# JialeTao/MRFA

Measured on AMD Instinct MI355X. Metric: frames/sec (256x256 source+driving pair) fwd+bwd, higher is better.
Workload: dtype f32; 1 GPU; vox1.yaml MTIA (TokenPose_B) prior + DenseMotion + RaftFlow refinement, 256x256, bs=8/GPU, fwd+bwd+clip+Adam, train-mode BN, surrogate L1 loss; global_batch=8, parallelism=dp1, prior=mtia, background_predictor=False, sync_bn=False, launch=hipGraph, optimizer=FlatAdam (K20), mfma=bf16x6

## Files before the change

### mrfa_amd/build.py

```python
import glob
import os
import subprocess
import sys

HERE = os.path.dirname(os.path.abspath(__file__))
ROOT = os.path.dirname(HERE)
CSRC = os.path.join(HERE, "csrc")
LIBDIR = os.path.join(HERE, "_lib")
LIB = os.path.join(LIBDIR, "libmrfa_hip.so")
SOURCES = ["error.cpp", "conv_plan.hip", "conv_mfma.hip", "conv_split.hip", "conv_halo.hip", "conv_small.hip", "conv_lean.hip", "wgrad_mfma.hip", "wgrad_split.hip", "wgrad_halo.hip", "wgrad_small.hip", "wgrad_lean.hip", "conv_fewout.hip", "conv_fewout3.hip", "layout.hip", "pack_multi.hip", "norm.hip", "sample.hip", "elementwise.hip", "optim.hip", "tokenpose.hip", "attention_mfma.hip", "losses.hip", "prior.hip", "pose.hip", "metrics.hip", "frames.hip"]
FLAGS = ["--offload-arch=gfx950", "-O3", "-std=c++17", "-fPIC", "-I" + os.path.join(ROOT, "include"), "-I" + CSRC,
         "-Wno-unused-result"]


def _stale(out, deps):
    if not os.path.exists(out):
        return True
    t = os.path.getmtime(out)
    return any(os.path.getmtime(d) > t for d in deps)


def build(force: bool = False, verbose: bool = True) -> str:
    os.makedirs(LIBDIR, exist_ok=True)
    hipcc = os.environ.get("HIPCC", "/opt/rocm/bin/hipcc")
    headers = [os.path.join(ROOT, "include", "mrfa_hip.h")] + sorted(glob.glob(os.path.join(CSRC, "*.h")))
    objs = []
    procs = []
    for src in SOURCES:
        sp = os.path.join(CSRC, src)
        if not os.path.exists(sp):
            raise FileNotFoundError(sp)
        obj = os.path.join(LIBDIR, os.path.splitext(src)[0] + ".o")
        objs.append(obj)
        if force or _stale(obj, [sp] + headers):
            cmd = [hipcc] + FLAGS + (["-x", "hip"] if src.endswith(".cpp") else []) + ["-c", sp, "-o", obj]
            if verbose:
                print("[mrfa_amd.build]", " ".join(cmd), flush=True)
            procs.append((src, subprocess.Popen(cmd)))
    for src, pr in procs:
        if pr.wait() != 0:
            raise RuntimeError(f"hipcc failed on {src}")
    if force or _stale(LIB, objs):
        cmd = [hipcc, "--offload-arch=gfx950", "-shared", "-fPIC", "-o", LIB] + objs
        if verbose:
            print("[mrfa_amd.build]", " ".join(cmd), flush=True)
        subprocess.check_call(cmd)
    return LIB


if __name__ == "__main__":
    build(force="--force" in sys.argv)
    print(LIB)
```

### mrfa_amd/csrc/common.h

```cpp
#pragma once
#include <hip/hip_runtime.h>
#include <stdio.h>
#include <string.h>
#include "mrfa_hip.h"

typedef float f32x16 __attribute__((ext_vector_type(16)));
typedef float f32x4 __attribute__((ext_vector_type(4)));

void mrfa_set_error(const char* fmt, ...);

struct MrfaTuning {
    int conv_small_env;
    int conv_small;
    int conv_halo, conv_halo_min_tiles, conv_halo_pr, conv_halo_phase, conv_halo_bn256, conv_halo_bn192, conv_halo_bn64_fill;
    int conv_lean, conv_lean_min_wgs, conv_lean_geo, gemm_lean;
    int wgrad_halo, wgrad_halo_min_wgs, wgrad_halo_target_wgs, wgrad_halo_phase, wgrad_lean;
    int conv_fewout3, attention_mfma, split_target_256;
};
extern MrfaTuning g_tune;

struct HaloGeo { int PR, BN; bool phase; };

enum class ConvFamily { lean, gemm_lean, small, halo, halo_dgrad, rows_split, rows_f32, refused };
struct ConvPlan {
    ConvFamily family;
    char error[256];
    long long M;
    int KT;
    int lean_geo, gemm_cfg, small_tm, small_tn;
    HaloGeo halo;
    int BM, BN, splitk;
    bool w8;
    bool fused;
    bool fin_in_launch;
    bool reads_w;
    int last_config;
    bool groups_ok, bst_ok, stride2_ok, mask_ok, phase_dgrad_ok;
};
ConvPlan plan_conv(const mrfa_conv_params& p);

enum class WgradFamily { lean, small, halo, tiled, refused };
struct WgradPlan {
    WgradFamily family;
    char error[192];
    long long M;
    bool lean, small;
    bool groups_ok, stride2_ok;
};
WgradPlan plan_wgrad(const mrfa_wgrad_params& p);

int mrfa_conv_split_launch(hipStream_t st, const mrfa_conv_params& p, int KT, long long M, int splitk, int BN);
bool mrfa_conv_halo_eligible(const mrfa_conv_params& p, HaloGeo* geo);
int mrfa_conv_halo_launch(hipStream_t st, const mrfa_conv_params& p, const HaloGeo& geo);
int mrfa_wgrad_split_launch(hipStream_t st, const mrfa_wgrad_params& p, dim3 grid, long long M, long long kps, int tiles_n, int nsplit, int inner,
                            int total_splits, int taps, long long partial_stride, int BM, int BN);

bool mrfa_wgrad_halo_eligible(const mrfa_wgrad_params& p);
int mrfa_wgrad_halo_launch(hipStream_t st, const mrfa_wgrad_params& p);

bool mrfa_fewout3_wgrad(hipStream_t st, const float* x, int ldx, int N, int H, int W, int Cin, const float* dy, int lddy, int Cout, int R, int pad,
                        float* dw, float* dbias, int* rc);

int mrfa_conv_lean_pick(const mrfa_conv_params& p);
int mrfa_conv_lean_launch(hipStream_t st, const mrfa_conv_params& p, int geo);
int mrfa_gemm_lean_pick(const mrfa_conv_params& p, long long M);
int mrfa_gemm_lean_launch(hipStream_t st, const mrfa_conv_params& p, long long M, int cfg);

bool mrfa_conv_small_eligible(const mrfa_conv_params& p, long long M);
int mrfa_conv_small_launch(hipStream_t st, const mrfa_conv_params& p, long long M, int tm, int tn);

bool mrfa_attention_mfma_ok(int d, int n, const void* qkv, int ld, const void* out, int ldo, const void* dout, int lddo, const void* dqkv, int lddq);
int mrfa_attention_fwd_mfma(hipStream_t st, const float* qkv, int ld, int B, int n, int heads, int d, float scale, float* out, int ldo, float* lse);
int mrfa_attention_bwd_mfma(hipStream_t st, const float* qkv, int ld, const float* out, int ldo, const float* dout, int lddo, const float* lse,
                            float* delta, int B, int n, int heads, int d, float scale, float* dqkv, int lddq);

bool mrfa_wgrad_lean_eligible(const mrfa_wgrad_params& p);
int mrfa_wgrad_lean_multi(hipStream_t st, const mrfa_wgrad_params* ps, int n, unsigned char* taken);

bool mrfa_wgrad_small_eligible(const mrfa_wgrad_params& p, long long M);
int mrfa_wgrad_small_launch(hipStream_t st, const mrfa_wgrad_params& p, long long M);

#define MRFA_CHECK_ARG(cond, ...)                      \
    do {                                               \
        if (!(cond)) {                                 \
            mrfa_set_error(__VA_ARGS__);               \
            return 1;                                  \
        }                                              \
    } while (0)

#define MRFA_CHECK_LAUNCH(name)                                                   \
    do {                                                                          \
        hipError_t e_ = hipGetLastError();                                        \
        if (e_ != hipSuccess) {                                                   \
            mrfa_set_error("%s: launch failed: %s", name, hipGetErrorString(e_)); \
            return 2;                                                             \
        }                                                                         \
    } while (0)

static inline bool aligned16(const void* p) { return (reinterpret_cast<uintptr_t>(p) & 15u) == 0; }
static inline int cdiv(long long a, long long b) { return (int)((a + b - 1) / b); }

static inline int stream_grid(long long work_items, int block) {
    long long g = (work_items + block - 1) / block;
    if (g < 1) g = 1;
    if (g > 256 * 16) g = 256 * 16;
    return (int)g;
}

__device__ __forceinline__ int xcd_tile_index() {
    const int per_xcd = (int)gridDim.x >> 3;
    return (int)(blockIdx.x & 7) * per_xcd + (int)(blockIdx.x >> 3);
}

__device__ __forceinline__ void chain_prio() {
    __builtin_amdgcn_s_setprio(3);
}

__device__ __forceinline__ int stat_group(const mrfa_conv_params& p, long long row, long long M) {
    return p.groups > 1 ? (int)(row / (M / p.groups)) : 0;
}
__device__ __forceinline__ double* stat_slot(const mrfa_conv_params& p, int group, unsigned slot) {
    return p.stats + ((size_t)group * MRFA_STATS_SLOTS + slot % MRFA_STATS_SLOTS) * 2 * p.Cout;
}
static inline long long group_rows(const mrfa_conv_params& p, long long M) {
    if (p.groups <= 1) return M;
    return (p.N % p.groups) == 0 ? M / p.groups : 0;
}

__device__ __forceinline__ bool splitk_last_arriver(unsigned* ticket, unsigned nsplit) {
    __shared__ unsigned s_sk_ticket;
    asm volatile("s_waitcnt vmcnt(0)" ::: "memory");
    __syncthreads();
    if (threadIdx.x == 0) s_sk_ticket = __hip_atomic_fetch_add(ticket, 1u, __ATOMIC_RELAXED, __HIP_MEMORY_SCOPE_AGENT);
    __syncthreads();
    return s_sk_ticket == nsplit - 1;
}

__device__ __forceinline__ bool fin_last_arriver(unsigned* counter, unsigned participants, int idx) {
    __shared__ unsigned s_fin_ticket;
    asm volatile("s_waitcnt vmcnt(0)" ::: "memory");
    __syncthreads();
    if (threadIdx.x == 0) {
        if (idx < 0) {
            s_fin_ticket = __hip_atomic_fetch_add(counter, 1u, __ATOMIC_RELAXED, __HIP_MEMORY_SCOPE_AGENT) == participants - 1;
        } else {
            const unsigned nsh = participants < 8u ? participants : 8u, sh = (unsigned)idx % nsh;
            const unsigned mine = participants / nsh + (sh < participants % nsh ? 1u : 0u);
            unsigned last = 0;
            if (__hip_atomic_fetch_add(counter + 1 + sh, 1u, __ATOMIC_RELAXED, __HIP_MEMORY_SCOPE_AGENT) == mine - 1)
                last = __hip_atomic_fetch_add(counter, 1u, __ATOMIC_RELAXED, __HIP_MEMORY_SCOPE_AGENT) == nsh - 1;
            s_fin_ticket = last;
        }
    }
    __syncthreads();
    return s_fin_ticket != 0;
}

__device__ __forceinline__ double fin_slot_sum(const double* first, size_t stride) {
    double v[MRFA_STATS_SLOTS];
#pragma unroll
    for (int s = 0; s < MRFA_STATS_SLOTS; ++s) v[s] = __hip_atomic_load(first + (size_t)s * stride, __ATOMIC_RELAXED, __HIP_MEMORY_SCOPE_AGENT);
    double t = 0.0;
#pragma unroll
    for (int s = 0; s < MRFA_STATS_SLOTS; ++s) t += v[s];
    return t;
}

__device__ __forceinline__ void fused_bn_finalize(const mrfa_conv_params& p, unsigned participants, int idx = -1, double* scratch = nullptr, int scratch_n = 0) {
    if (!fin_last_arriver(p.fin_counter, participants, idx)) return;
    const double cnt = (double)p.fin_count;
    const int G = p.groups > 1 ? p.groups : 1;
    const int C2 = 2 * p.Cout;
    const bool par = scratch != nullptr && scratch_n >= G * C2;
    if (par) {
        for (int o = threadIdx.x; o < G * C2; o += blockDim.x) scratch[o] = fin_slot_sum(p.stats + (size_t)(o / C2) * MRFA_STATS_SLOTS * C2 + o % C2, (size_t)C2);
        __syncthreads();
    }
    for (int c = threadIdx.x; c < p.Cout; c += blockDim.x) {
        float rm = p.fin_rmean ? p.fin_rmean[c] : 0.f, rv = p.fin_rmean ? p.fin_rvar[c] : 0.f;
        for (int g = 0; g < G; ++g) {
            const double* sg = p.stats + (size_t)g * MRFA_STATS_SLOTS * C2;
            const double t1 = par ? scratch[g * C2 + c] : fin_slot_sum(sg + c, (size_t)C2);
            const double t2 = par ? scratch[g * C2 + p.Cout + c] : fin_slot_sum(sg + p.Cout + c, (size_t)C2);
            const double m = t1 / cnt;
            double var = t2 / cnt - m * m;
            if (var < 0.0) var = 0.0;
            const float mean = (float)m, invstd = (float)(1.0 / sqrt(var + (double)p.fin_eps));
            const double unb = p.fin_count > 1 ? var * cnt / (cnt - 1.0) : var;
            rm = (1.f - p.fin_momentum) * rm + p.fin_momentum * mean;
            rv = (1.f - p.fin_momentum) * rv + p.fin_momentum * (float)unb;
            const float sc = p.fin_gamma[c] * invstd;
            const int gc = g * p.Cout + c;
            p.fin_scale[gc] = sc;
            p.fin_shift[gc] = p.fin_beta[c] - mean * sc;
            if (p.fin_mean) p.fin_mean[gc] = mean;
            if (p.fin_invstd) p.fin_invstd[gc] = invstd;
        }
        if (p.fin_rmean) { p.fin_rmean[c] = rm; p.fin_rvar[c] = rv; }
    }
}

__device__ __forceinline__ float wave_sum(float v) {
#pragma unroll
    for (int o = 32; o > 0; o >>= 1) v += __shfl_xor(v, o, 64);
    return v;
}
```

### mrfa_amd/csrc/conv_mfma.hip

```cpp
#include "common.h"
#include <stdlib.h>

namespace {

constexpr int BK = 32;
constexpr int LDK = BK + 4;

template <int BM, int BN, int WAVES_M, int WAVES_N, bool FLAT>
__global__ __launch_bounds__(WAVES_M * WAVES_N * 64) void conv_mfma_kernel(const mrfa_conv_params p, const int KT, const int kt_per_split,
                                                       const long long M, const int tiles_n, const int total_tiles) {
    constexpr int TM = BM / WAVES_M / 32;
    constexpr int TN = BN / WAVES_N / 32;
    constexpr int NT = WAVES_M * WAVES_N * 64;
    constexpr int RSTEP = NT / 8;
    constexpr int RA = BM / RSTEP;
    constexpr int RB = BN / RSTEP;
    static_assert(WAVES_M * WAVES_N == 4 || WAVES_M * WAVES_N == 8, "4 or 8 waves");
    static_assert(RA >= 1 && RB >= 1, "tile too small for the workgroup");
    static_assert(TM >= 1 && TN >= 1, "tile");

    __shared__ __attribute__((aligned(16))) float smem[2 * (BM + BN) * LDK];

    const int tid = threadIdx.x;
    const int lane = tid & 63;
// ... 35 lines not shown
    bool b_ok[RB];
#pragma unroll
    for (int j = 0; j < RB; ++j) b_ok[j] = (n0 + lrow + RSTEP * j) < p.w_rows;

    f32x4 ra[RA], rb[RB];

    int l_r = 0, l_s = 0, l_c = 0;
    const float* l_w = w;
    const int a_koff = kq * 4;

    auto load_tiles = [&](int kt) {
        if constexpr (!FLAT) {
            const int c0 = l_c * 32 + a_koff;
            f32x4 sc = {1.f, 1.f, 1.f, 1.f}, sh = {0.f, 0.f, 0.f, 0.f};
            if (p.in_scale) {
                sc = *reinterpret_cast<const f32x4*>(p.in_scale + c0);
                sh = *reinterpret_cast<const f32x4*>(p.in_shift + c0);
            }
            const int dr = l_r - p.pad, ds = l_s - p.pad;
#pragma unroll
            for (int j = 0; j < RA; ++j) {
                const int iy = a_oy[j] + dr;
                const int ix = a_ox[j] + ds;
                const bool inb = a_ok[j] && (unsigned)iy < (unsigned)Hv && (unsigned)ix < (unsigned)Wv;
                const int pix = inb ? (a_base[j] + (iy >> p.ups) * p.Win + (ix >> p.ups)) : a_base[j];
                f32x4 v = *reinterpret_cast<const f32x4*>(x + (size_t)pix * p.ldx + c0);
                if (p.in_scale) {
                    v = v * sc + sh;
                    if (p.in_relu) {
                        v.x = fmaxf(v.x, 0.f); v.y = fmaxf(v.y, 0.f); v.z = fmaxf(v.z, 0.f); v.w = fmaxf(v.w, 0.f);
                    }
                }
                ra[j] = inb ? v : f32x4{0.f, 0.f, 0.f, 0.f};
            }
            const float* wt = l_w + c0;
#pragma unroll
            for (int j = 0; j < RB; ++j) {
                const int row = b_ok[j] ? (n0 + lrow + RSTEP * j) : 0;
                const f32x4 v = *reinterpret_cast<const f32x4*>(wt + (size_t)row * p.w_ld);
                rb[j] = b_ok[j] ? v : f32x4{0.f, 0.f, 0.f, 0.f};
            }
            if (++l_c == KC) {
                l_c = 0;
                l_w += p.w_tap;
                if (++l_s == p.S) { l_s = 0; ++l_r; }
            }
        } else {
            const int k0 = kt * 32 + kq * 4;
            const int4 ent = *reinterpret_cast<const int4*>(p.ktab + k0);
            const int e[4] = {ent.x, ent.y, ent.z, ent.w};
#pragma unroll
            for (int j = 0; j < RA; ++j) {
                float vv[4];
#pragma unroll
                for (int q = 0; q < 4; ++q) {
                    float v = 0.f;
                    if (e[q] >= 0 && a_ok[j]) {
                        const int dy = (e[q] & 255) - 128, dx = ((e[q] >> 8) & 255) - 128, ci = e[q] >> 16;
                        const int iy = a_oy[j] + dy, ix = a_ox[j] + dx;
                        if ((unsigned)iy < (unsigned)Hv && (unsigned)ix < (unsigned)Wv) {
                            const size_t pix = (size_t)(a_base[j] + (iy >> p.ups) * p.Win + (ix >> p.ups));
                            v = x[pix * p.ldx + ci];
                            if (p.in_scale) {
                                v = v * p.in_scale[ci] + p.in_shift[ci];
                                if (p.in_relu) v = fmaxf(v, 0.f);
                            }
                        }
                    }
                    vv[q] = v;
                }
                ra[j] = f32x4{vv[0], vv[1], vv[2], vv[3]};
            }
#pragma unroll
            for (int j = 0; j < RB; ++j) {
                f32x4 v = {0.f, 0.f, 0.f, 0.f};
                if (b_ok[j]) v = *reinterpret_cast<const f32x4*>(w + (size_t)(n0 + lrow + RSTEP * j) * p.w_ld + k0);
                rb[j] = v;
            }
        }
    };

    auto store_tiles = [&](int buf) {
        float* As = smem + buf * (BM + BN) * LDK;
        float* Bs = As + BM * LDK;
#pragma unroll
        for (int j = 0; j < RA; ++j) *reinterpret_cast<f32x4*>(As + (lrow + RSTEP * j) * LDK + kq * 4) = ra[j];
#pragma unroll
        for (int j = 0; j < RB; ++j) *reinterpret_cast<f32x4*>(Bs + (lrow + RSTEP * j) * LDK + kq * 4) = rb[j];
    };

    f32x16 acc[TM][TN];
#pragma unroll
    for (int i = 0; i < TM; ++i)
#pragma unroll
        for (int j = 0; j < TN; ++j)
#pragma unroll
            for (int r = 0; r < 16; ++r) acc[i][j][r] = 0.f;

    const int kt_begin = blockIdx.z * kt_per_split;
    const int kt_end = min(KT, kt_begin + kt_per_split);

    if constexpr (!FLAT) {
        const int tap0 = kt_begin / KC;
        l_c = kt_begin - tap0 * KC;
        l_r = tap0 / p.S;
        l_s = tap0 - l_r * p.S;
        l_w = w + (size_t)tap0 * p.w_tap;
    }
    if (kt_begin < kt_end) {
        load_tiles(kt_begin);
        store_tiles(0);
    }
    __syncthreads();

    const int frag_row = lane & 31;
    const int frag_k = (lane >> 5) * 4;
    int cur = 0;
    for (int kt = kt_begin; kt < kt_end; ++kt) {
        const bool more = (kt + 1) < kt_end;
        if (more) load_tiles(kt + 1);
        const float* As = smem + cur * (BM + BN) * LDK + (wm * TM * 32 + frag_row) * LDK + frag_k;
        const float* Bs = smem + cur * (BM + BN) * LDK + BM * LDK + (wn * TN * 32 + frag_row) * LDK + frag_k;
#pragma unroll
        for (int q = 0; q < 4; ++q) {
            f32x4 a[TM], b[TN];
#pragma unroll
            for (int i = 0; i < TM; ++i) a[i] = *reinterpret_cast<const f32x4*>(As + i * 32 * LDK + q * 8);
#pragma unroll
            for (int j = 0; j < TN; ++j) b[j] = *reinterpret_cast<const f32x4*>(Bs + j * 32 * LDK + q * 8);
#pragma unroll
            for (int e = 0; e < 4; ++e)
#pragma unroll
                for (int i = 0; i < TM; ++i)
#pragma unroll
                    for (int j = 0; j < TN; ++j)
                        acc[i][j] = __builtin_amdgcn_mfma_f32_32x32x2f32(a[i][e], b[j][e], acc[i][j], 0, 0, 0);
        }
        if (more) store_tiles(cur ^ 1);
        __syncthreads();
        cur ^= 1;
    }

    const int half = lane >> 5;
    const bool splitk = p.splitk > 1;
    if (splitk) {
#pragma unroll
        for (int j = 0; j < TN; ++j) {
            const int c = n0 + (wn * TN + j) * 32 + (lane & 31);
#pragma unroll
            for (int i = 0; i < TM; ++i)
#pragma unroll
                for (int r = 0; r < 16; ++r) {
                    const long long m = m0 + (wm * TM + i) * 32 + (r & 3) + 8 * (r >> 2) + 4 * half;
                    if (c < p.Cout && m < M) atomicAdd(y + (size_t)m * p.ldy + c, acc[i][j][r] * p.alpha);
                }
        }
        if (!p.sk_ticket || !splitk_last_arriver(p.sk_ticket + (size_t)bz * total_tiles + lin, gridDim.z)) return;
    }
#pragma unroll
    for (int j = 0; j < TN; ++j) {
        const int c = n0 + (wn * TN + j) * 32 + (lane & 31);
        const bool c_ok = c < p.Cout;
        float bias = 0.f, osc = 1.f, osh = 0.f;
        if (c_ok) {
            if (p.bias) bias = p.bias[c];
            if (p.out_scale) { osc = p.out_scale[c]; osh = p.out_shift[c]; }
        }
        float s1 = 0.f, s2 = 0.f;
        const int cq = c_ok ? c : 0;
#pragma unroll
        for (int i = 0; i < TM; ++i) {
            float yv[16], rv[16];
            auto row_of = [&](int r) {
                const long long m = m0 + (wm * TM + i) * 32 + (r & 3) + 8 * (r >> 2) + 4 * half;
                return m < M ? m : M - 1;
            };
            if (splitk) {
#pragma unroll
                for (int r = 0; r < 16; ++r) yv[r] = __hip_atomic_load(y + (size_t)row_of(r) * p.ldy + cq, __ATOMIC_RELAXED, __HIP_MEMORY_SCOPE_AGENT);
            } else if (p.accumulate) {
#pragma unroll
                for (int r = 0; r < 16; ++r) yv[r] = y[(size_t)row_of(r) * p.ldy + cq];
            } else {
#pragma unroll
                for (int r = 0; r < 16; ++r) yv[r] = 0.f;
            }
            if (p.res) {
#pragma unroll
                for (int r = 0; r < 16; ++r) rv[r] = p.res[(size_t)row_of(r) * p.ldr + cq];
            } else {
#pragma unroll
                for (int r = 0; r < 16; ++r) rv[r] = 0.f;
            }
#pragma unroll
            for (int r = 0; r < 16; ++r) {
                const long long m = m0 + (wm * TM + i) * 32 + (r & 3) + 8 * (r >> 2) + 4 * half;
                if (c_ok && m < M) {
                    float* dst = y + (size_t)m * p.ldy + c;
                    float v = splitk ? yv[r] : acc[i][j][r] * p.alpha;
                    v += bias;
                    v = v * osc + osh;
                    v += rv[r];
                    if (p.relu) v = fmaxf(v, 0.f);
                    if (!splitk) v += yv[r];
                    *dst = v;
                    s1 += v;
                    s2 += v * v;
                }
            }
        }
        if (p.stats) {
            s1 += __shfl_xor(s1, 32, 64);
            s2 += __shfl_xor(s2, 32, 64);
            if (half == 0 && c_ok) {
                double* st = stat_slot(p, stat_group(p, m0, M), blockIdx.x);
                atomicAdd(st + c, (double)s1);
                atomicAdd(st + p.Cout + c, (double)s2);
            }
        }
    }
    if (p.fin_scale) fused_bn_finalize(p, (unsigned)total_tiles);
}

__global__ void splitk_init_kernel(float* y, int ldy, long long rows, int C, const float* bias) {
    const long long total = rows * C;
    for (long long i = blockIdx.x * (long long)blockDim.x + threadIdx.x; i < total; i += (long long)gridDim.x * blockDim.x) {
        const long long r = i / C;
        const int c = (int)(i - r * C);
        y[(size_t)r * ldy + c] = bias ? bias[c] : 0.f;
    }
}

__global__ void splitk_epilogue_kernel(float* y, int ldy, long long rows, int C, const float* osc, const float* osh,
                                       const float* res, int ldr, int relu, double* stats) {
    const int c = blockIdx.x * blockDim.x + threadIdx.x;
    if (c >= C) return;
    const float sc = osc ? osc[c] : 1.f, sh = osh ? osh[c] : 0.f;
    float s1 = 0.f, s2 = 0.f;
    for (long long r = blockIdx.y; r < rows; r += gridDim.y) {
        float v = y[(size_t)r * ldy + c] * sc + sh;
        if (res) v += res[(size_t)r * ldr + c];
        if (relu) v = fmaxf(v, 0.f);
        y[(size_t)r * ldy + c] = v;
        s1 += v;
        s2 += v * v;
    }
    if (stats) {
        double* st = stats + (size_t)(blockIdx.y % MRFA_STATS_SLOTS) * 2 * C;
        atomicAdd(st + c, (double)s1);
        atomicAdd(st + C + c, (double)s2);
    }
}

template <int BM, int BN, int WM_, int WN_>
int launch_cfg(hipStream_t st, const mrfa_conv_params& p, int KT, long long M, int splitk) {
    const int tiles_n = cdiv(p.Cout, BN);
    const long long tiles_m = (M + BM - 1) / BM;
    const int total_tiles = (int)(tiles_m * tiles_n);
    dim3 grid((unsigned)(cdiv(total_tiles, 8) * 8), (unsigned)(p.nbatch > 1 ? p.nbatch : 1), (unsigned)splitk);
    const int kps = cdiv(KT, splitk);
    mrfa_conv_params q = p;
    q.splitk = splitk;
    if (p.kflat > 0)
        hipLaunchKernelGGL((conv_mfma_kernel<BM, BN, WM_, WN_, true>), grid, dim3(WM_ * WN_ * 64), 0, st, q, KT, kps, M, tiles_n, total_tiles);
    else
        hipLaunchKernelGGL((conv_mfma_kernel<BM, BN, WM_, WN_, false>), grid, dim3(WM_ * WN_ * 64), 0, st, q, KT, kps, M, tiles_n, total_tiles);
    MRFA_CHECK_LAUNCH("mrfa_conv2d_nhwc");
    return 0;
}

}

static int g_mfma_mode = 0;
extern "C" int mrfa_set_mfma_mode(int mode) {
    if (mode < 0 || mode > 3) { mrfa_set_error("set_mfma_mode: unknown mode %d", mode); return 1; }
    g_mfma_mode = mode;
    return 0;
}
extern "C" int mrfa_get_mfma_mode(void) { return g_mfma_mode; }

static thread_local int g_last_tile = 0;
extern "C" int mrfa_conv2d_last_config(void) { return g_last_tile; }

static int launch_rows(hipStream_t st, const mrfa_conv_params& p, const ConvPlan& c) {
    const bool flat = p.kflat > 0;
    const long long M = c.M;
    const int nb = p.nbatch > 1 ? p.nbatch : 1;
    const int splitk = c.splitk;
    mrfa_conv_params pk = p;
    if (splitk > 1) {
        const bool init = !p.accumulate && !(p.y_zero && (c.fused || !p.bias));
        if (init) {
            const long long rows = M * nb;
            MRFA_CHECK_ARG(nb == 1 || p.y_bs == (long long)M * p.ldy, "conv2d: split-K batched output must be dense");
            hipLaunchKernelGGL(splitk_init_kernel, dim3(stream_grid(rows * p.Cout, 256)), dim3(256), 0, st, p.y, p.ldy, rows,
                               p.Cout, p.bias);
            MRFA_CHECK_LAUNCH("splitk_init");
            pk.bias = nullptr;
        }
        if (!c.fused) pk.sk_ticket = nullptr;
    }
    if (!c.fin_in_launch) pk.fin_scale = nullptr;
    g_last_tile = c.last_config;
    const int BM = c.BM, BN = c.BN;
    int rc = 1;
#define CFG(bm, bn, wm, wn) if (BM == bm && BN == bn) rc = launch_cfg<bm, bn, wm, wn>(st, pk, c.KT, M, splitk)
    if (c.family == ConvFamily::rows_split) rc = mrfa_conv_split_launch(st, pk, c.KT, M, splitk, BN);
    else if (c.w8 && BM == 128 && BN == 128) rc = launch_cfg<128, 128, 2, 4>(st, pk, c.KT, M, splitk);
    else CFG(128, 128, 2, 2);
    else CFG(128, 96, 4, 1);
    else CFG(128, 64, 2, 2);
    else CFG(128, 32, 4, 1);
    else CFG(64, 128, 2, 2);
    else CFG(64, 64, 2, 2);
    else CFG(32, 128, 1, 4);
    else { mrfa_set_error("conv2d: no tile config %dx%d", BM, BN); return 1; }
#undef CFG
    if (rc) return rc;
    if (splitk > 1 && !c.fused && (p.relu || p.stats || p.out_scale || p.res)) {
        MRFA_CHECK_ARG(!p.accumulate, "conv2d: split-K with accumulate cannot apply an epilogue");
        const long long rows = M * nb;
        dim3 grid(cdiv(p.Cout, 64), (unsigned)(rows < 256 ? rows : 256));
        hipLaunchKernelGGL(splitk_epilogue_kernel, grid, dim3(64), 0, st, p.y, p.ldy, rows, p.Cout, p.out_scale, p.out_shift,
                           p.res, p.ldr, p.relu, p.stats);
        MRFA_CHECK_LAUNCH("splitk_epilogue");
    }
    return 0;
}

extern "C" int mrfa_conv2d_nhwc(void* stream, const mrfa_conv_params* pp) {
    MRFA_CHECK_ARG(pp, "conv2d: null parameter block");
    const mrfa_conv_params& p = *pp;
    hipStream_t st = (hipStream_t)stream;
    const ConvPlan c = plan_conv(p);
    MRFA_CHECK_ARG(c.groups_ok, "conv2d: groups = %d is not implemented for these parameters (N = %d, %d x %d outputs, splitk %d): ask "
                   "mrfa_conv2d_groups_supported() first", p.groups, p.N, p.Hout, p.Wout, p.splitk);
    if (p.fin_scale) {
        MRFA_CHECK_ARG(p.stats && p.fin_shift && p.fin_gamma && p.fin_beta && p.fin_counter && p.fin_count > 0,
                       "conv2d: fin_scale needs stats, fin_shift, fin_gamma, fin_beta, fin_counter and fin_count > 0");
        MRFA_CHECK_ARG((p.fin_rmean == nullptr) == (p.fin_rvar == nullptr), "conv2d: fin_rmean / fin_rvar come together");
    }
    if (p.bst_x) {
        MRFA_CHECK_ARG(p.stats && p.bst_scale && p.bst_shift && p.bst_mean && p.bst_invstd && !p.fin_scale,
                       "conv2d: bst_x needs stats, bst_scale / _shift / _mean / _invstd and no fin_*");
        MRFA_CHECK_ARG(c.bst_ok, "conv2d: bst_* is only implemented by the small-problem kernels: ask mrfa_conv2d_bwdstats_supported() first");
    }
    MRFA_CHECK_ARG(p.y, "conv2d: null pointer");
    if (c.family == ConvFamily::refused) { mrfa_set_error("%s", c.error); return 1; }
    int rc;
    switch (c.family) {
        case ConvFamily::lean: g_last_tile = c.last_config; rc = mrfa_conv_lean_launch(st, p, c.lean_geo); break;
        case ConvFamily::gemm_lean: g_last_tile = c.last_config; rc = mrfa_gemm_lean_launch(st, p, c.M, c.gemm_cfg); break;
        case ConvFamily::small: g_last_tile = c.last_config; rc = mrfa_conv_small_launch(st, p, c.M, c.small_tm, c.small_tn); break;
        case ConvFamily::halo:
        case ConvFamily::halo_dgrad: g_last_tile = c.last_config; rc = mrfa_conv_halo_launch(st, p, c.halo); break;
        default: rc = launch_rows(st, p, c); break;
    }
    if (rc || !p.fin_scale || c.fin_in_launch) return rc;
    return mrfa_bn_finalize_groups(stream, p.stats, p.fin_count, p.fin_gamma, p.fin_beta, p.fin_rmean, p.fin_rvar, p.fin_momentum, p.fin_eps,
                                   p.Cout, p.groups > 1 ? p.groups : 1, p.fin_scale, p.fin_shift, p.fin_mean, p.fin_invstd);
}
```

### mrfa_amd/csrc/conv_plan.hip

```cpp
#include "common.h"
#include <stdarg.h>
#include <stdlib.h>

namespace {
int env_int(const char* name, int dflt) { const char* e = getenv(name); return e ? atoi(e) : dflt; }
int env_on(const char* name) { const char* e = getenv(name); return !(e && e[0] == '0'); }
}

MrfaTuning g_tune = {
     env_on("MRFA_CONV_SMALL"),  1,
     env_on("MRFA_CONV_HALO"),  128,  0,  1,  1,
     1,  1,
     env_on("MRFA_CONV_LEAN"),  128,  -1,
     env_int("MRFA_GEMM_LEAN", 1),
     env_on("MRFA_WGRAD_HALO"),  192,  256,  1,
     env_on("MRFA_WGRAD_LEAN"),
     1,  env_on("MRFA_ATTENTION_MFMA"),  env_int("MRFA_SPLIT_TARGET_256", 1),
};

enum TuneKind { T_ON, T_INT, T_NONNEG, T_NONNEG_ON, T_LEVEL, T_POS };
static const struct { const char* key; int* field; TuneKind kind; } TUNING_KEYS[] = {
    {"conv_small", &g_tune.conv_small, T_ON},
    {"conv_halo", &g_tune.conv_halo, T_ON},
    {"conv_halo_min_tiles", &g_tune.conv_halo_min_tiles, T_INT},
    {"conv_halo_pr", &g_tune.conv_halo_pr, T_INT},
    {"conv_halo_phase", &g_tune.conv_halo_phase, T_ON},
    {"conv_halo_bn256", &g_tune.conv_halo_bn256, T_ON},
    {"conv_halo_bn192", &g_tune.conv_halo_bn192, T_ON},
    {"conv_halo_bn64_fill", &g_tune.conv_halo_bn64_fill, T_ON},
    {"conv_lean", &g_tune.conv_lean, T_ON},
    {"conv_lean_min_wgs", &g_tune.conv_lean_min_wgs, T_NONNEG},
    {"conv_lean_geo", &g_tune.conv_lean_geo, T_INT},
    {"gemm_lean", &g_tune.gemm_lean, T_LEVEL},
    {"wgrad_halo", &g_tune.wgrad_halo, T_ON},
    {"wgrad_halo_min_wgs", &g_tune.wgrad_halo_min_wgs, T_NONNEG},
    {"wgrad_halo_target_wgs", &g_tune.wgrad_halo_target_wgs, T_POS},
    {"wgrad_halo_phase", &g_tune.wgrad_halo_phase, T_NONNEG_ON},
    {"wgrad_lean", &g_tune.wgrad_lean, T_ON},
    {"conv_fewout3", &g_tune.conv_fewout3, T_ON},
    {"attention_mfma", &g_tune.attention_mfma, T_ON},
};

extern "C" int mrfa_set_tuning(const char* key, int value) {
    if (!key) return -1;
    for (const auto& k : TUNING_KEYS) {
        if (strcmp(key, k.key)) continue;
        const int prev = *k.field;
        switch (k.kind) {
            case T_ON: *k.field = value != 0; break;
            case T_INT: *k.field = value; break;
            case T_NONNEG: if (value >= 0) *k.field = value; break;
            case T_NONNEG_ON: if (value >= 0) *k.field = value != 0; break;
            case T_LEVEL: if (value >= 0) *k.field = value > 2 ? 2 : value; break;
            case T_POS: if (value > 0) *k.field = value; break;
        }
        return prev;
    }
    return -1;
}

namespace {
constexpr int BK = 32;

template <typename Plan>
Plan& refuse(Plan& c, const char* fmt, ...) {
    va_list ap;
    va_start(ap, fmt);
    vsnprintf(c.error, sizeof(c.error), fmt, ap);
    va_end(ap);
    c.family = decltype(c.family)::refused;
    return c;
}

void plan_rows(ConvPlan& c, const mrfa_conv_params& p, int mode) {
    const bool flat = p.kflat > 0;
    const long long M = c.M;
    const int KT = c.KT;
    const int nb = p.nbatch > 1 ? p.nbatch : 1;
    int BN = 128;
    {
        const int cands[4] = {128, 96, 64, 32};
        const double pen[4] = {1.0, 1.08, 1.16, 1.3};
        double best = 1e18;
        for (int i = 0; i < 4; ++i) {
            if (cands[i] == 96 && flat) continue;
            const double cost = (double)cdiv(p.Cout, cands[i]) * cands[i] * pen[i];
            if (cost < best) { best = cost; BN = cands[i]; }
        }
    }
    if (mode >= 1 && !flat && p.Cout >= 32) BN = p.Cout <= 64 ? 64 : 128;
    auto ntiles = [&](int bm, int bn) { return ((M + bm - 1) / bm) * cdiv(p.Cout, bn) * nb; };
    int BM = 128;
    if (BN == 96 && ntiles(128, 96) < 384) BN = 128;
    if (BN == 128) { if (M <= 32) BM = 32; else if (M <= 64) BM = 64; }
    else if (BN == 64 && M <= 64) BM = 64;
    int splitk = 1;
    const bool auto_split = (p.splitk == 0);
    if (p.splitk > 1) splitk = p.splitk;
    {
        const bool short_k_big_m = KT < 32 && M > 4096;
        const bool grouped_stats = p.groups > 1 && p.stats && !(p.sk_ticket && !p.accumulate);
        const int max_split = (auto_split && !short_k_big_m && !grouped_stats) ? (KT / 2 > 0 ? KT / 2 : 1) : 1;
        long long t = ntiles(BM, BN);
        if (t < 384 && !(short_k_big_m && t >= 128)) {
            const bool half_target = g_tune.split_target_256 && auto_split && p.sk_ticket && !p.accumulate && KT >= 72 && KT <= 320 && BM == 128 && t >= 8 && t <= 16;
            int want = (int)(((half_target ? 256 : 512) + t - 1) / t);
            if (auto_split) splitk = want <= max_split ? want : max_split;
            const int min_bm = (BN == 128) ? 32 : (BN == 64 ? 64 : 128);
            while (!half_target && ntiles(BM, BN) * splitk < 384 && BM > min_bm) {
                BM >>= 1;
                if (auto_split) {
                    t = ntiles(BM, BN);
                    want = (int)((512 + t - 1) / t);
                    splitk = want <= max_split ? want : max_split;
                }
            }
            if (splitk < 1) splitk = 1;
        }
    }
    bool w8 = false;
    if (p.tile) {
        BM = p.tile >> 16; BN = p.tile & 0x7fff; w8 = (p.tile & 0x8000) != 0;
        if (p.splitk >= 1) splitk = p.splitk;
    } else if (BM == 128 && BN == 128 && !flat) {
        w8 = true;
    }
    const bool split_operand = mode >= 1 && BM == 128 && (BN == 128 || BN == 64) && !flat;
    c.family = split_operand ? ConvFamily::rows_split : ConvFamily::rows_f32;
    c.BM = BM;
    c.BN = BN;
    c.w8 = w8;
    c.splitk = splitk;
    c.fused = splitk > 1 && p.sk_ticket && !p.accumulate;
    c.fin_in_launch = p.fin_scale && nb == 1 && (splitk == 1 || c.fused);
    c.reads_w = !(split_operand && mode != 3 && p.w_split);
    c.last_config = (BM << 16) | (BN << 4) | ((flat ? 1 : 0) << 1) | (splitk > 1 ? 1 : 0) | (split_operand ? 4 : 0);
}
}

ConvPlan plan_conv(const mrfa_conv_params& p) {
    ConvPlan c = {};
    const int mode = mrfa_get_mfma_mode();
    const bool flat = p.kflat > 0;
    c.M = (long long)p.N * p.Hout * p.Wout;
    c.KT = ((flat ? p.kflat : p.R * p.S * p.Cin) + BK - 1) / BK;
    c.splitk = 1;
    c.reads_w = true;
    c.fin_in_launch = p.fin_scale != nullptr;

    c.lean_geo = flat ? -1 : mrfa_conv_lean_pick(p);
    c.gemm_cfg = (flat || c.lean_geo >= 0) ? -1 : mrfa_gemm_lean_pick(p, c.M);
    const bool lean = c.lean_geo >= 0, gemm = c.gemm_cfg >= 0;
    const bool small = !lean && !gemm && g_tune.conv_small_env && g_tune.conv_small && mrfa_conv_small_eligible(p, c.M);
    const bool halo = !flat && mrfa_conv_halo_eligible(p, &c.halo);

    const long long rows = group_rows(p, c.M);
    c.groups_ok = p.groups <= 1 || !(p.stats || p.fin_scale || p.bst_x || p.in_scale) ||
                  (p.nbatch <= 1 && p.splitk <= 1 && rows > 0 &&
                   (lean || gemm || (!p.in_scale && ((rows % 128) == 0 || small || (p.stride <= 1 && halo)))));
    c.bst_ok = p.stats && !p.fin_scale && p.stride >= 0 && !flat && (lean || gemm || small);
    c.stride2_ok = p.stride == 2 && p.Hout == (p.Hin + 2 * p.pad - p.R) / 2 + 1 && p.Wout == (p.Win + 2 * p.pad - p.S) / 2 + 1 &&
                   (flat ? (!p.ups && p.nbatch <= 1 && p.splitk <= 1 && p.ktab) : small);
    c.mask_ok = halo;
    c.phase_dgrad_ok = p.ups == 2 && halo;

    if (!(p.x && p.w)) return refuse(c, "conv2d: null pointer");
    if (!(p.N > 0 && p.Cin > 0 && p.Cout > 0 && p.Hout > 0 && p.Wout > 0)) return refuse(c, "conv2d: bad sizes");
    if (!(p.R >= 1 && p.S >= 1 && p.R <= 15 && p.S <= 15)) return refuse(c, "conv2d: kernel size %dx%d unsupported", p.R, p.S);
    if (!((p.w_ld % 4) == 0 && aligned16(p.w))) return refuse(c, "conv2d: packed weight must be 16-B aligned, w_ld %% 4 == 0");
    if (!flat && (p.Cin % 32) != 0) return refuse(c, "conv2d: chunked mode needs Cin %% 32 == 0 (got %d); use flat mode", p.Cin);
    if (!flat && !((p.ldx % 4) == 0 && aligned16(p.x))) return refuse(c, "conv2d: chunked mode needs 16-B aligned x and ldx %% 4 == 0");
    if (!flat && p.in_scale && !(aligned16(p.in_scale) && aligned16(p.in_shift))) return refuse(c, "conv2d: in_scale/in_shift alignment");
    if (flat && !(p.ktab != nullptr && aligned16(p.ktab))) return refuse(c, "conv2d: flat mode needs a 16-B aligned ktab");
    if (lean) {
        c.family = ConvFamily::lean;
        c.reads_w = false;
        c.last_config = (32 << 16) | (32 << 4) | 4 | (1 << 27);
        return c;
    }
    if (gemm) {
        c.family = ConvFamily::gemm_lean;
        c.reads_w = false;
        c.last_config = (64 << 16) | (64 << 4) | 4 | (1 << 26);
        return c;
    }
    if (small) {
        c.family = ConvFamily::small;
        const int ncols = (p.Cout + 15) / 16 * 16;
        auto waves = [&](int wm, int wn) { return ((c.M + wm - 1) / wm) * ((ncols + wn - 1) / wn); };
        int tm = 2, tn = 2;
        if (waves(32, 32) < 2048) { tm = 1; tn = 2; }
        if (tm == 1 && waves(16, 32) < 2048) { tn = 1; }
        if (ncols % 32 != 0 && tn == 2 && ncols < 32) tn = 1;
        if (p.groups > 1 && tm == 2 && (rows % 128) != 0) tm = 1;
        c.small_tm = tm;
        c.small_tn = tn;
        c.last_config = (16 << 16) | (16 << 4) | 8;
        return c;
    }
    if (p.stride < 0 || p.stride > 2 || (p.stride == 2 && !(flat && !p.ups && p.nbatch <= 1)))
        return refuse(c, "conv2d: stride = %d is only implemented by the one-wave-per-tile kernel and by flat-K launches: ask mrfa_conv2d_stride_supported() first", p.stride);
    if (p.mask && !halo) return refuse(c, "conv2d: `mask` is only honoured by the patch-tiled kernel: ask mrfa_conv2d_mask_supported() first");
    if (p.ups == 2 && !halo)
        return refuse(c, "conv2d: ups = 2 (phase data gradient of a fused-upsample layer) is only implemented for the shapes mrfa_conv2d_phase_dgrad_supported() reports");
    if (halo) {
        c.family = p.ups == 2 ? ConvFamily::halo_dgrad : ConvFamily::halo;
        c.reads_w = false;
        c.last_config = (128 << 16) | ((p.Cout <= 64 ? 64 : 128) << 4) | 4 | (1 << 28);
        return c;
    }
    plan_rows(c, p, mode);
    return c;
}

WgradPlan plan_wgrad(const mrfa_wgrad_params& p) {
    WgradPlan c = {};
    const bool flat = p.kflat > 0;
    c.M = (long long)p.N * p.Hout * p.Wout;
    c.lean = mrfa_wgrad_lean_eligible(p);
    c.small = g_tune.conv_small_env && g_tune.conv_small && mrfa_wgrad_small_eligible(p, c.M);
    c.groups_ok = p.groups <= 1 || !p.in_scale || c.lean;
    c.stride2_ok = p.stride == 2 && p.Hout == (p.Hin + 2 * p.pad - p.R) / 2 + 1 && p.Wout == (p.Win + 2 * p.pad - p.S) / 2 + 1 && c.small;
    if (!(p.x && p.dy && p.dw)) return refuse(c, "wgrad: null pointer");
    if (!flat && !((p.ldx % 4) == 0 && aligned16(p.x))) return refuse(c, "wgrad: x must be a 16-B aligned view with ld %% 4 == 0");
    if (flat && !p.ktab) return refuse(c, "wgrad: flat mode needs ktab");
    if (!(c.M < (1ll << 31) - 64)) return refuse(c, "wgrad: too many pixels");
    if (p.in_scale && c.lean) { c.family = WgradFamily::lean; return c; }
    if (!c.groups_ok) return refuse(c, "wgrad: groups = %d with a prologue is only implemented where mrfa_conv2d_wgrad_groups_supported() says so", p.groups);
    if (c.small) { c.family = WgradFamily::small; return c; }
    if (p.stride > 1) return refuse(c, "wgrad: stride = %d is only implemented by the small-problem kernel: ask mrfa_conv2d_wgrad_stride_supported() first", p.stride);
    c.family = !flat && mrfa_wgrad_halo_eligible(p) ? WgradFamily::halo : WgradFamily::tiled;
    return c;
}

extern "C" int mrfa_conv2d_split_k(const mrfa_conv_params* p) {
    if (!p) return 1;
    if (p->splitk > 1) return p->splitk;
    const ConvPlan c = plan_conv(*p);
    return c.family == ConvFamily::refused ? 1 : c.splitk;
}

extern "C" int mrfa_conv2d_reads_fp32_weights(const mrfa_conv_params* p) {
    if (!p) return 1;
    const ConvPlan c = plan_conv(*p);
    return c.family == ConvFamily::refused || c.reads_w ? 1 : 0;
}

extern "C" int mrfa_conv2d_groups_supported(const mrfa_conv_params* p) { return p && plan_conv(*p).groups_ok ? 1 : 0; }
extern "C" int mrfa_conv2d_bwdstats_supported(const mrfa_conv_params* p) { return p && plan_conv(*p).bst_ok ? 1 : 0; }
extern "C" int mrfa_conv2d_stride_supported(const mrfa_conv_params* p) { return p && plan_conv(*p).stride2_ok ? 1 : 0; }
extern "C" int mrfa_conv2d_mask_supported(const mrfa_conv_params* p) { return p && plan_conv(*p).mask_ok ? 1 : 0; }
extern "C" int mrfa_conv2d_phase_dgrad_supported(const mrfa_conv_params* p) { return p && plan_conv(*p).phase_dgrad_ok ? 1 : 0; }

extern "C" int mrfa_conv2d_wgrad_stride_supported(const mrfa_wgrad_params* p) { return p && plan_wgrad(*p).stride2_ok ? 1 : 0; }
extern "C" int mrfa_conv2d_wgrad_groups_supported(const mrfa_wgrad_params* p) { return p && plan_wgrad(*p).groups_ok ? 1 : 0; }
extern "C" int mrfa_conv2d_wgrad_lean_supported(const mrfa_wgrad_params* p) { return p && plan_wgrad(*p).lean ? 1 : 0; }
```

Measured before the change: 101.1 pairs/s.

## Add deep-K split convolution kernel for small-M, large-K fused split-K convs

Adds a new convolution kernel for layers with few output pixels and a deep reduction (R*S*Cin). It splits K across waves and workgroups, register-pipelines the loads in a four-deep ring, and reduces within the workgroup through LDS. Results are combined across workgroups with atomics, and the last arriver applies the fused bias, BN, residual and ReLU epilogue and the stats. The goal is to use more CUs on the small, deep layers that the row-tiled split-K path runs with little parallelism. The cost is float atomics, which make results non-deterministic, plus a global re-read in the epilogue.

```diff
diff --git a/mrfa_amd/build.py b/mrfa_amd/build.py
--- a/mrfa_amd/build.py
+++ b/mrfa_amd/build.py
@@ -8,7 +8,7 @@
 CSRC = os.path.join(HERE, "csrc")
 LIBDIR = os.path.join(HERE, "_lib")
 LIB = os.path.join(LIBDIR, "libmrfa_hip.so")
-SOURCES = ["error.cpp", "conv_plan.hip", "conv_mfma.hip", "conv_split.hip", "conv_halo.hip", "conv_small.hip", "conv_lean.hip", "wgrad_mfma.hip", "wgrad_split.hip", "wgrad_halo.hip", "wgrad_small.hip", "wgrad_lean.hip", "conv_fewout.hip", "conv_fewout3.hip", "layout.hip", "pack_multi.hip", "norm.hip", "sample.hip", "elementwise.hip", "optim.hip", "tokenpose.hip", "attention_mfma.hip", "losses.hip", "prior.hip", "pose.hip", "metrics.hip", "frames.hip"]
+SOURCES = ["error.cpp", "conv_plan.hip", "conv_mfma.hip", "conv_split.hip", "conv_halo.hip", "conv_small.hip", "conv_lean.hip", "conv_deepk.hip", "wgrad_mfma.hip", "wgrad_split.hip", "wgrad_halo.hip", "wgrad_small.hip", "wgrad_lean.hip", "conv_fewout.hip", "conv_fewout3.hip", "layout.hip", "pack_multi.hip", "norm.hip", "sample.hip", "elementwise.hip", "optim.hip", "tokenpose.hip", "attention_mfma.hip", "losses.hip", "prior.hip", "pose.hip", "metrics.hip", "frames.hip"]
 FLAGS = ["--offload-arch=gfx950", "-O3", "-std=c++17", "-fPIC", "-I" + os.path.join(ROOT, "include"), "-I" + CSRC,
          "-Wno-unused-result"]
 
diff --git a/mrfa_amd/csrc/common.h b/mrfa_amd/csrc/common.h
--- a/mrfa_amd/csrc/common.h
+++ b/mrfa_amd/csrc/common.h
@@ -16,12 +16,14 @@
     int conv_lean, conv_lean_min_wgs, conv_lean_geo, gemm_lean;
     int wgrad_halo, wgrad_halo_min_wgs, wgrad_halo_target_wgs, wgrad_halo_phase, wgrad_lean;
     int conv_fewout3, attention_mfma, split_target_256;
+    int conv_deepk;
 };
 extern MrfaTuning g_tune;
 
 struct HaloGeo { int PR, BN; bool phase; };
-
-enum class ConvFamily { lean, gemm_lean, small, halo, halo_dgrad, rows_split, rows_f32, refused };
+struct DeepkGeo { int MT, NT, nslice, steps_per_wave; };
+
+enum class ConvFamily { lean, gemm_lean, small, halo, halo_dgrad, deepk, rows_split, rows_f32, refused };
 struct ConvPlan {
     ConvFamily family;
     char error[256];
@@ -29,6 +31,7 @@
     int KT;
     int lean_geo, gemm_cfg, small_tm, small_tn;
     HaloGeo halo;
+    DeepkGeo deepk;
     int BM, BN, splitk;
     bool w8;
     bool fused;
@@ -52,6 +55,8 @@
 int mrfa_conv_split_launch(hipStream_t st, const mrfa_conv_params& p, int KT, long long M, int splitk, int BN);
 bool mrfa_conv_halo_eligible(const mrfa_conv_params& p, HaloGeo* geo);
 int mrfa_conv_halo_launch(hipStream_t st, const mrfa_conv_params& p, const HaloGeo& geo);
+bool mrfa_conv_deepk_eligible(const mrfa_conv_params& p, long long M, int level, DeepkGeo* geo);
+int mrfa_conv_deepk_launch(hipStream_t st, const mrfa_conv_params& p, long long M, const DeepkGeo& geo);
 int mrfa_wgrad_split_launch(hipStream_t st, const mrfa_wgrad_params& p, dim3 grid, long long M, long long kps, int tiles_n, int nsplit, int inner,
                             int total_splits, int taps, long long partial_stride, int BM, int BN);
 
diff --git a/mrfa_amd/csrc/conv_deepk.hip b/mrfa_amd/csrc/conv_deepk.hip
--- /dev/null
+++ b/mrfa_amd/csrc/conv_deepk.hip
@@ -0,0 +1,332 @@
+#include "mfma_bf16.h"
+
+namespace {
+
+template <int MT, int NT, int NP, bool PRO>
+__global__ __launch_bounds__(256) void conv_deepk_kernel(const mrfa_conv_params p, const long long M, const int ncol, const int nslice, const int steps_total,
+                                                         const int steps_per_wave, const int nstrips) {
+    constexpr int NPC = NP == 6 ? 3 : (NP == 3 ? 2 : 1);
+    constexpr int NB = NP == 1 ? 2 : NPC;
+    constexpr int RING = 4;
+    constexpr int TL = MT * NT;
+    __shared__ float red[4 * 3 * TL * 4 * 64];
+    __shared__ float s_st[4][2][32 * NT];
+
+    const int tid = threadIdx.x, lane = tid & 63, wave = __builtin_amdgcn_readfirstlane(tid >> 6);
+    const int px = lane & 31, half = lane >> 5;
+    const int id = (int)blockIdx.x;
+    const int col = id % ncol;
+    const int slice = (id / ncol) % nslice;
+    const int rs = id / (ncol * nslice);
+    const long long m0 = (long long)rs * (32 * MT);
+    const int n0 = col * (32 * NT);
+    const int T = p.R * p.S;
+    const int Hv = p.Hin << p.ups, Wv = p.Win << p.ups;
+    const int HWo = p.Hout * p.Wout;
+
+    const int q = slice * 4 + wave;
+    const int s_begin = min(q * steps_per_wave, steps_total);
+    const int s_end = min(s_begin + steps_per_wave, steps_total);
+
+    int a_oy[MT], a_ox[MT], a_base[MT];
+    bool a_ok[MT];
+#pragma unroll
+    for (int i = 0; i < MT; ++i) {
+        const long long m = m0 + i * 32 + px;
+        a_ok[i] = m < M;
+        const long long mm = a_ok[i] ? m : 0;
+        const int n_img = (int)(mm / HWo);
+        const int rem = (int)(mm - (long long)n_img * HWo);
+        a_oy[i] = rem / p.Wout;
+        a_ox[i] = rem - a_oy[i] * p.Wout;
+        a_base[i] = n_img * p.Hin * p.Win;
+    }
+
+    f32x4 ra[RING][MT][2], psc[RING][2], psh[RING][2];
+    u32x4 rb[RING][NT][NB];
+    unsigned a_inb[RING];
+    int l_step = min(s_begin, steps_total - 1);
+    const int l_last = max(s_end - 1, l_step);
+    int l_c = l_step / T;
+    int l_tap = l_step - l_c * T;
+    int l_r = l_tap / p.S, l_s = l_tap - l_r * p.S;
+    const unsigned short* __restrict__ ws = reinterpret_cast<const unsigned short*>(p.w_split) + (size_t)(n0 + px) * 16 + half * 8;
+    const float* __restrict__ wf = p.w + (size_t)(n0 + px) * p.w_ld + half * 8;
+    const size_t chunk_stride = (size_t)p.w_rows * 16;
+
+    auto issue = [&](int slot) {
+        const int c0 = l_c * 16 + half * 8;
+        const int dr = l_r - p.pad, ds = l_s - p.pad;
+        unsigned inb_bits = 0;
+#pragma unroll
+        for (int i = 0; i < MT; ++i) {
+            const int iy = a_oy[i] + dr, ix = a_ox[i] + ds;
+            const bool inb = a_ok[i] && (unsigned)iy < (unsigned)Hv && (unsigned)ix < (unsigned)Wv;
+            const int pix = inb ? (a_base[i] + (iy >> p.ups) * p.Win + (ix >> p.ups)) : a_base[i];
+            const float* src = p.x + (size_t)pix * p.ldx + c0;
+            ra[slot][i][0] = *reinterpret_cast<const f32x4*>(src);
+            ra[slot][i][1] = *reinterpret_cast<const f32x4*>(src + 4);
+            inb_bits |= (inb ? 1u : 0u) << i;
+        }
+        a_inb[slot] = inb_bits;
+        if constexpr (PRO) {
+#pragma unroll
+            for (int h = 0; h < 2; ++h) {
+                psc[slot][h] = *reinterpret_cast<const f32x4*>(p.in_scale + c0 + 4 * h);
+                psh[slot][h] = *reinterpret_cast<const f32x4*>(p.in_shift + c0 + 4 * h);
+            }
+        }
+#pragma unroll
+        for (int j = 0; j < NT; ++j) {
+            if constexpr (NP == 1) {
+                const float* src = wf + (size_t)l_tap * p.w_tap + (size_t)j * 32 * p.w_ld + l_c * 16;
+                rb[slot][j][0] = *reinterpret_cast<const u32x4*>(src);
+                rb[slot][j][1] = *reinterpret_cast<const u32x4*>(src + 4);
+            } else {
+                const unsigned short* src = ws + (size_t)l_tap * p.w_tap + (size_t)l_c * chunk_stride + j * (32 * 16);
+#pragma unroll
+                for (int pc = 0; pc < NPC; ++pc) rb[slot][j][pc] = *reinterpret_cast<const u32x4*>(src + (size_t)pc * p.w_piece);
+            }
+        }
+        if (l_step < l_last) {
+            ++l_step;
+            ++l_tap;
+            if (++l_s == p.S) {
+                l_s = 0;
+                if (++l_r == p.R) { l_r = 0; l_tap = 0; ++l_c; }
+            }
+        }
+    };
+
+    f32x16 acc[TL][2];
+#pragma unroll
+    for (int i = 0; i < TL; ++i)
+#pragma unroll
+        for (int k = 0; k < 2; ++k)
+#pragma unroll
+            for (int r = 0; r < 16; ++r) acc[i][k][r] = 0.f;
+
+    auto split = [&](int slot, bf16x8 (&a)[3][MT]) {
+        const f32x4 z = {0.f, 0.f, 0.f, 0.f};
+#pragma unroll
+        for (int i = 0; i < MT; ++i) {
+            u32x2 pl[3], ph[3];
+            f32x4 v0 = ra[slot][i][0], v1 = ra[slot][i][1];
+            if constexpr (PRO) {
+                v0 = v0 * psc[slot][0] + psh[slot][0];
+                v1 = v1 * psc[slot][1] + psh[slot][1];
+#pragma unroll
+                for (int e = 0; e < 4; ++e) { v0[e] = fmaxf(v0[e], 0.f); v1[e] = fmaxf(v1[e], 0.f); }
+            }
+            const bool inb = (a_inb[slot] >> i) & 1u;
+            v0 = inb ? v0 : z;
+            v1 = inb ? v1 : z;
+            bf16_pieces<NP>(v0, pl[0], pl[1], pl[2]);
+            bf16_pieces<NP>(v1, ph[0], ph[1], ph[2]);
+#pragma unroll
+            for (int pc = 0; pc < NPC; ++pc) a[pc][i] = __builtin_bit_cast(bf16x8, u32x4{pl[pc][0], pl[pc][1], ph[pc][0], ph[pc][1]});
+        }
+    };
+    auto mfma_step = [&](int slot, const bf16x8 (&a)[3][MT]) {
+        bf16x8 b[NT][3];
+#pragma unroll
+        for (int j = 0; j < NT; ++j) {
+            if constexpr (NP == 1) {
+                const f32x4 w0 = __builtin_bit_cast(f32x4, rb[slot][j][0]), w1 = __builtin_bit_cast(f32x4, rb[slot][j][1]);
+                u32x2 bl, bh, u2, u3;
+                bf16_pieces<1>(w0, bl, u2, u3);
+                bf16_pieces<1>(w1, bh, u2, u3);
+                b[j][0] = __builtin_bit_cast(bf16x8, u32x4{bl[0], bl[1], bh[0], bh[1]});
+            } else {
+#pragma unroll
+                for (int pc = 0; pc < NPC; ++pc) b[j][pc] = __builtin_bit_cast(bf16x8, rb[slot][j][pc]);
+            }
+        }
+#pragma unroll
+        for (int t = 6 - NP; t < 6; ++t)
+#pragma unroll
+            for (int i = 0; i < MT; ++i)
+#pragma unroll
+                for (int j = 0; j < NT; ++j)
+                    acc[i * NT + j][t < 3 ? 1 : 0] = __builtin_amdgcn_mfma_f32_32x32x16_bf16(a[PA[t]][i], b[j][PB[t]], acc[i * NT + j][t < 3 ? 1 : 0], 0, 0, 0);
+    };
+
+#pragma unroll
+    for (int u = 0; u < RING; ++u) issue(u);
+    bf16x8 a_cur[3][MT], a_nxt[3][MT];
+    split(0, a_cur);
+    for (int s = s_begin; s < s_end; s += RING) {
+#pragma unroll
+        for (int u = 0; u < RING; ++u) {
+            if (s + u < s_end) {
+                split((u + 1) % RING, a_nxt);
+                mfma_step(u, a_cur);
+                issue(u);
+#pragma unroll
+                for (int pc = 0; pc < 3; ++pc)
+#pragma unroll
+                    for (int i = 0; i < MT; ++i) a_cur[pc][i] = a_nxt[pc][i];
+            }
+        }
+    }
+
+#pragma unroll
+    for (int i = 0; i < TL; ++i)
+#pragma unroll
+        for (int r = 0; r < 16; ++r) acc[i][0][r] += acc[i][1][r];
+#pragma unroll
+    for (int o = 0; o < 4; ++o) {
+        if (o != wave) {
+            const int k = wave < o ? wave : wave - 1;
+#pragma unroll
+            for (int i = 0; i < TL; ++i)
+#pragma unroll
+                for (int e = 0; e < 4; ++e) red[(((o * 3 + k) * TL + i) * 4 + e) * 64 + lane] = acc[i][0][4 * o + e];
+        }
+    }
+    __syncthreads();
+    float v[TL][4];
+#pragma unroll
+    for (int o = 0; o < 4; ++o) {
+        if (o == wave) {
+#pragma unroll
+            for (int i = 0; i < TL; ++i)
+#pragma unroll
+                for (int e = 0; e < 4; ++e) {
+                    float t = acc[i][0][4 * o + e];
+#pragma unroll
+                    for (int k = 0; k < 3; ++k) t += red[(((o * 3 + k) * TL + i) * 4 + e) * 64 + lane];
+                    v[i][e] = t;
+                }
+        }
+    }
+
+    float* __restrict__ y = p.y;
+    auto row_of = [&](int i, int e) { return m0 + i * 32 + 8 * wave + 4 * half + e; };
+#pragma unroll
+    for (int i = 0; i < MT; ++i)
+#pragma unroll
+        for (int j = 0; j < NT; ++j)
+#pragma unroll
+            for (int e = 0; e < 4; ++e) {
+                const long long m = row_of(i, e);
+                const int c = n0 + j * 32 + px;
+                if (c < p.Cout && m < M) atomicAdd(y + (size_t)m * p.ldy + c, v[i * NT + j][e] * p.alpha);
+            }
+    if (!splitk_last_arriver(p.sk_ticket + (size_t)rs * ncol + col, (unsigned)nslice)) return;
+
+    float yv[TL][4], rv[TL][4], bias[NT], osc[NT], osh[NT];
+#pragma unroll
+    for (int j = 0; j < NT; ++j) {
+        const int c = n0 + j * 32 + px, cq = c < p.Cout ? c : 0;
+        bias[j] = p.bias ? p.bias[cq] : 0.f;
+        osc[j] = p.out_scale ? p.out_scale[cq] : 1.f;
+        osh[j] = p.out_scale ? p.out_shift[cq] : 0.f;
+#pragma unroll
+        for (int i = 0; i < MT; ++i)
+#pragma unroll
+            for (int e = 0; e < 4; ++e) {
+                const long long m = row_of(i, e);
+                const long long mc = m < M ? m : M - 1;
+                yv[i * NT + j][e] = __hip_atomic_load(y + (size_t)mc * p.ldy + cq, __ATOMIC_RELAXED, __HIP_MEMORY_SCOPE_AGENT);
+                rv[i * NT + j][e] = p.res ? p.res[(size_t)mc * p.ldr + cq] : 0.f;
+            }
+    }
+    float s1[NT], s2[NT];
+#pragma unroll
+    for (int j = 0; j < NT; ++j) {
+        const int c = n0 + j * 32 + px;
+        s1[j] = s2[j] = 0.f;
+#pragma unroll
+        for (int i = 0; i < MT; ++i)
+#pragma unroll
+            for (int e = 0; e < 4; ++e) {
+                const long long m = row_of(i, e);
+                if (c < p.Cout && m < M) {
+                    float u = yv[i * NT + j][e] + bias[j];
+                    u = u * osc[j] + osh[j];
+                    u += rv[i * NT + j][e];
+                    if (p.relu) u = fmaxf(u, 0.f);
+                    y[(size_t)m * p.ldy + c] = u;
+                    s1[j] += u;
+                    s2[j] += u * u;
+                }
+            }
+    }
+    if (p.stats) {
+#pragma unroll
+        for (int j = 0; j < NT; ++j) {
+            s1[j] += __shfl_xor(s1[j], 32, 64);
+            s2[j] += __shfl_xor(s2[j], 32, 64);
+            if (half == 0) { s_st[wave][0][j * 32 + px] = s1[j]; s_st[wave][1][j * 32 + px] = s2[j]; }
+        }
+        __syncthreads();
+        if (tid < 64 * NT) {
+            const int which = tid / (32 * NT), ch = tid % (32 * NT);
+            const float t = (s_st[0][which][ch] + s_st[1][which][ch]) + (s_st[2][which][ch] + s_st[3][which][ch]);
+            if (n0 + ch < p.Cout)
+                atomicAdd(stat_slot(p, stat_group(p, m0, M), blockIdx.x) + which * p.Cout + n0 + ch, (double)t);
+        }
+        if (p.fin_scale) fused_bn_finalize(p, (unsigned)nstrips);
+    }
+}
+
+template <int MT, int NT, int NP>
+void launch_pro(hipStream_t st, const mrfa_conv_params& p, dim3 grid, long long M, int ncol, int nslice, int steps, int spw, int nstrips) {
+    if (p.in_scale) hipLaunchKernelGGL((conv_deepk_kernel<MT, NT, NP, true>), grid, dim3(256), 0, st, p, M, ncol, nslice, steps, spw, nstrips);
+    else hipLaunchKernelGGL((conv_deepk_kernel<MT, NT, NP, false>), grid, dim3(256), 0, st, p, M, ncol, nslice, steps, spw, nstrips);
+}
+template <int MT, int NT>
+void launch_np(hipStream_t st, const mrfa_conv_params& p, dim3 grid, long long M, int ncol, int nslice, int steps, int spw, int nstrips) {
+    const int mode = mrfa_get_mfma_mode();
+    if (mode == 3) launch_pro<MT, NT, 1>(st, p, grid, M, ncol, nslice, steps, spw, nstrips);
+    else if (mode == 2) launch_pro<MT, NT, 3>(st, p, grid, M, ncol, nslice, steps, spw, nstrips);
+    else launch_pro<MT, NT, 6>(st, p, grid, M, ncol, nslice, steps, spw, nstrips);
+}
+
+}
+
+bool mrfa_conv_deepk_eligible(const mrfa_conv_params& p, long long M, int level, DeepkGeo* geo) {
+    const int mode = mrfa_get_mfma_mode();
+    if (level <= 0 || (mode != 1 && mode != 2 && mode != 3)) return false;
+    if (p.kflat > 0 || !p.sk_ticket || p.accumulate || p.nbatch > 1 || p.tile || p.mask || p.bst_x) return false;
+    if (p.stride > 1 || p.stride < 0 || p.ups < 0 || p.ups > 1) return false;
+    if ((p.Cin % 32) != 0 || (p.ldx % 4) != 0 || !aligned16(p.x)) return false;
+    if (mode != 3 && (!p.w_split || p.w_piece <= 0)) return false;
+    if (mode == 3 && ((p.w_ld % 4) != 0 || !aligned16(p.w))) return false;
+    if (p.in_scale && (!p.in_relu || p.groups > 1 || !aligned16(p.in_scale) || !aligned16(p.in_shift))) return false;
+    if (M >= (1ll << 31) - 128 || (long long)p.N * p.Hin * p.Win >= (1ll << 31)) return false;
+    const int MT = M > 32 ? 2 : 1, NT = (MT == 2 && p.Cout > 32) ? 2 : 1;
+    if (p.w_rows < cdiv(p.Cout, 32 * NT) * 32 * NT) return false;
+    if (p.groups > 1 && (p.stats || p.fin_scale) && (group_rows(p, M) % (32 * MT)) != 0) return false;
+    const int steps = p.R * p.S * (p.Cin / 16);
+    const int ncol = cdiv(p.Cout, 32 * NT);
+    const long long strips = (long long)cdiv(M, 32 * MT) * ncol;
+    int nslice;
+    if (p.splitk > 1) {
+        nslice = p.splitk;
+    } else {
+        nslice = (int)(256 / strips);
+        if (nslice > 8) nslice = 8;
+        if (nslice > steps / 8) nslice = steps / 8;
+        if (nslice < 1) nslice = 1;
+    }
+    if (strips * nslice > (1 << 20)) return false;
+    if (level == 1) {
+        if (M > 2048 || 2.0 * (double)M * p.Cout * 16.0 * steps > 12e9) return false;
+    }
+    *geo = {MT, NT, nslice, cdiv(steps, nslice * 4)};
+    return true;
+}
+
+int mrfa_conv_deepk_launch(hipStream_t st, const mrfa_conv_params& p, long long M, const DeepkGeo& geo) {
+    const int steps = p.R * p.S * (p.Cin / 16);
+    const int ncol = cdiv(p.Cout, 32 * geo.NT);
+    const int nstrips = cdiv(M, 32 * geo.MT) * ncol;
+    dim3 grid((unsigned)(nstrips * geo.nslice));
+    if (geo.MT == 2 && geo.NT == 2) launch_np<2, 2>(st, p, grid, M, ncol, geo.nslice, steps, geo.steps_per_wave, nstrips);
+    else if (geo.MT == 2) launch_np<2, 1>(st, p, grid, M, ncol, geo.nslice, steps, geo.steps_per_wave, nstrips);
+    else launch_np<1, 1>(st, p, grid, M, ncol, geo.nslice, steps, geo.steps_per_wave, nstrips);
+    MRFA_CHECK_LAUNCH("mrfa_conv2d_nhwc(deepk)");
+    return 0;
+}
diff --git a/mrfa_amd/csrc/conv_mfma.hip b/mrfa_amd/csrc/conv_mfma.hip
--- a/mrfa_amd/csrc/conv_mfma.hip
+++ b/mrfa_amd/csrc/conv_mfma.hip
@@ -361,6 +361,7 @@
     }
     if (!c.fin_in_launch) pk.fin_scale = nullptr;
     g_last_tile = c.last_config;
+    if (c.family == ConvFamily::deepk) return mrfa_conv_deepk_launch(st, pk, M, c.deepk);
     const int BM = c.BM, BN = c.BN;
     int rc = 1;
 #define CFG(bm, bn, wm, wn) if (BM == bm && BN == bn) rc = launch_cfg<bm, bn, wm, wn>(st, pk, c.KT, M, splitk)
diff --git a/mrfa_amd/csrc/conv_plan.hip b/mrfa_amd/csrc/conv_plan.hip
--- a/mrfa_amd/csrc/conv_plan.hip
+++ b/mrfa_amd/csrc/conv_plan.hip
@@ -16,6 +16,7 @@
      env_on("MRFA_WGRAD_HALO"),  192,  256,  1,
      env_on("MRFA_WGRAD_LEAN"),
      1,  env_on("MRFA_ATTENTION_MFMA"),  env_int("MRFA_SPLIT_TARGET_256", 1),
+     env_int("MRFA_CONV_DEEPK", 1),
 };
 
 enum TuneKind { T_ON, T_INT, T_NONNEG, T_NONNEG_ON, T_LEVEL, T_POS };
@@ -39,6 +40,7 @@
     {"wgrad_lean", &g_tune.wgrad_lean, T_ON},
     {"conv_fewout3", &g_tune.conv_fewout3, T_ON},
     {"attention_mfma", &g_tune.attention_mfma, T_ON},
+    {"conv_deepk", &g_tune.conv_deepk, T_LEVEL},
 };
 
 extern "C" int mrfa_set_tuning(const char* key, int value) {
@@ -210,6 +212,10 @@
         return c;
     }
     plan_rows(c, p, mode);
+    if (c.fused && !flat && mrfa_conv_deepk_eligible(p, c.M, g_tune.conv_deepk, &c.deepk)) {
+        c.family = ConvFamily::deepk;
+        c.last_config = ((32 * c.deepk.MT) << 16) | (32 << 4) | 4 | 1 | (1 << 25);
+    }
     return c;
 }
 
```

Result: no change. 102.2 pairs/s, median of 4 (+1.0%).
